# simon-ging/coot-videotext

Measured on AMD Instinct MI355X. Metric: clip-pairs/sec (COOT retrieval train step, whole job), higher is better.
Workload: dtype bf16; 1 GPU; ActivityNet-shaped paper config (anet_coot): 64 videos x 4 clips per GPU, Lc=Lv=80, Ls=16, Lp=64, Dv=2048, Dt=1536, d_model=384; global_batch_videos=64, parallelism=dp1, mode=train, launch=native, deterministic=True, batches=two different synthetic batches in turn

## Files before the change

coot-videotext_amd/csrc/api.hip:

```cpp
#include <stdarg.h>
#include <stdio.h>
#include <string.h>

#include <algorithm>
#include <mutex>
#include <string>
#include <unordered_map>
#include <vector>

#include "../../include/coot_hip.h"
#include "attention.h"
#include "common.h"
#include "fused.h"
#include "gemm.h"
#include "loss.h"
#include "pool.h"
#include "ref_f32.h"
#include "rowops.h"

namespace coot {

static thread_local char g_err[512] = "";
static thread_local hipStream_t g_glob_flush_stream = nullptr;
static thread_local hipEvent_t g_glob_flush_ev = nullptr;
// ... 555 lines not shown
static LayerBufs self_bufs(const LayerS& s, int D) {
  LayerBufs b; b.q = s.qkv; b.ldq = 3 * D; b.k = s.qkv + D; b.ldk = 3 * D; b.v = s.qkv + 2 * D; b.ldv = 3 * D;
  b.ctx = s.ctx; b.r1 = s.r1; b.z1 = s.z1; b.h1 = s.h1; b.a1 = s.a1; b.r2 = s.r2; b.z2 = s.z2; b.lse = s.lse;
  return b;
}
static LayerBufs ctx_bufs(const CtxS& s, int D) {
  LayerBufs b; b.q = s.q; b.ldq = D; b.k = s.kv; b.ldk = 2 * D; b.v = s.kv + D; b.ldv = 2 * D;
  b.ctx = s.cctx; b.r1 = s.r1; b.z1 = s.z1; b.h1 = s.h1; b.a1 = s.a1; b.r2 = s.r2; b.z2 = s.z2; b.lse = s.lse;
  return b;
}

}

using namespace coot;

extern "C" {

const char* coot_last_error(void) { return coot::g_err; }
int coot_version(void) { return COOT_ABI_VERSION; }
int coot_debug_dropout_scales(uint64_t seed, unsigned site, uint64_t idx0, int64_t n, float p, float* out_host) {
  COOT_REQUIRE(out_host && n >= 0 && p > 0.f, "debug_dropout_scales: bad arguments");
  const DropCfg d = mkdrop(1, p, seed, site);
  const unsigned key = drop_key(seed, site);
  for (int64_t i = 0; i < n; ++i) out_host[i] = drop_scale_key(key, idx0 + (uint64_t)i, d.thr, d.inv_keep);
  return 0;
}
int coot_debug_attn_dropout_scales(uint64_t seed, unsigned site, unsigned row32, int Lk, float p, float* out_host) {
  COOT_REQUIRE(out_host && Lk >= 0 && p > 0.f, "debug_attn_dropout_scales: bad arguments");
  const DropCfg d = mkdrop(1, p, seed, site);
  const unsigned key = drop_key(seed, site);
  for (int k = 0; k < Lk; ++k) out_host[k] = attn_drop_scale(key, row32, k, (unsigned)(Lk + 1) >> 1, d.thr, d.inv_keep);
  return 0;
}
int coot_debug_timestamps(void* dev_u64) { g_fz_tstamps = (unsigned long long*)dev_u64; return 0; }
extern "C" void coot_step_stamps_enable(int on);
extern "C" void coot_step_grad_write(int on);
extern "C" void coot_step_det_seg_flush(int on);
extern "C" int coot_step_det_seg_flush_get(void);
extern "C" int coot_internal_stage_hits(void);
extern "C" void coot_step_text_ahead(int on);
extern "C" int coot_step_text_ahead_get(void);
extern "C" int coot_internal_text_ahead_steps(void);
extern "C" int coot_internal_stream_counter(int which);
extern "C++" { namespace coot { int det_bypass_count(); int det_overflow_count(); int det_set_overflow_guard(int on); int det_overflow_guard(); } }
extern "C++" { namespace coot { void set_rt_topk_splits(int n); int get_rt_topk_splits(); void set_rt_few_splits(int n); int get_rt_few_splits(); void set_rt_grouped_splits(int n); int get_rt_grouped_splits(); void set_rt_knn_splits(int n); int get_rt_knn_splits(); void set_rt_comp_blocks_per_wg(int n); int get_rt_comp_blocks_per_wg(); } }
int coot_get_option(const char* name, int* value) {
  if (!value) { set_error("get_option: null result"); return -1; }
  if (!strcmp(name, "tn_dma")) { *value = get_tn_dma(); return 0; }
  if (!strcmp(name, "xcd_order")) { *value = get_xcd_order(); return 0; }
  if (!strcmp(name, "tn_mode")) { *value = get_tn_mode(); return 0; }
  if (!strcmp(name, "stage_hits")) { *value = coot_internal_stage_hits(); return 0; }
  if (!strcmp(name, "text_ahead")) { *value = coot_step_text_ahead_get(); return 0; }
  if (!strcmp(name, "text_ahead_steps")) { *value = coot_internal_text_ahead_steps(); return 0; }
  if (!strcmp(name, "fused_attn_launches")) { *value = fused_attn_launches(); return 0; }
  if (!strcmp(name, "stream_overlap_tests")) { *value = coot_internal_stream_counter(0); return 0; }
  if (!strcmp(name, "stream_candidates_rejected")) { *value = coot_internal_stream_counter(1); return 0; }
  if (!strcmp(name, "stream_unresolved")) { *value = coot_internal_stream_counter(2); return 0; }
  if (!strcmp(name, "operand_f16")) { *value = COOT_OPERAND_IS_F16; return 0; }
  if (!strcmp(name, "det_seg_flush")) { *value = coot_step_det_seg_flush_get(); return 0; }
  if (!strcmp(name, "det_bypasses")) { *value = det_bypass_count(); return 0; }
  if (!strcmp(name, "det_overflows")) { *value = det_overflow_count(); return 0; }
  if (!strcmp(name, "det_overflow_check")) { *value = det_overflow_guard(); return 0; }
  if (!strcmp(name, "rt_topk_splits")) { *value = get_rt_topk_splits(); return 0; }
  if (!strcmp(name, "rt_few_splits")) { *value = get_rt_few_splits(); return 0; }
  if (!strcmp(name, "rt_grouped_splits")) { *value = get_rt_grouped_splits(); return 0; }
  if (!strcmp(name, "rt_knn_splits")) { *value = get_rt_knn_splits(); return 0; }
  if (!strcmp(name, "rt_comp_blocks_per_wg")) { *value = get_rt_comp_blocks_per_wg(); return 0; }
  set_error("get_option: unknown or write-only option %s", name);
  return -2;
}
int coot_set_option(const char* name, int value) {
  if (!strcmp(name, "tn_mode")) { set_tn_mode(value); return 0; }
  if (!strcmp(name, "step_stamps")) { coot_step_stamps_enable(value); return 0; }
  if (!strcmp(name, "fused")) { g_use_fused = value; return 0; }
  if (!strcmp(name, "glob_fused")) { g_use_glob_fused = value; return 0; }
  if (!strcmp(name, "glob_fused_bwd")) { g_use_glob_fused_bwd = value; return 0; }
  if (!strcmp(name, "packed")) { g_use_packed = value; return 0; }
  if (!strcmp(name, "fused_infc")) { g_use_fused_infc = value; return 0; }
  if (!strcmp(name, "fused_attn")) { set_fused_attn(value); return 0; }
  if (!strcmp(name, "tn_dma")) { set_tn_dma(value); return 0; }
  if (!strcmp(name, "pack_lazy")) { g_pack_lazy = value; return 0; }
  if (!strcmp(name, "pack_poison")) { g_pack_poison = value; return 0; }
  if (!strcmp(name, "grad_poison")) { g_grad_poison = value; return 0; }
  if (!strcmp(name, "tn_target_wgs")) { set_tn_target_wgs(value); return 0; }
  if (!strcmp(name, "xcd_order")) { set_xcd_order(value); return 0; }
  if (!strcmp(name, "grad_write")) { coot_step_grad_write(value); return 0; }
  if (!strcmp(name, "det_seg_flush")) { coot_step_det_seg_flush(value); return 0; }
  if (!strcmp(name, "text_ahead")) { coot_step_text_ahead(value); return 0; }
  if (!strcmp(name, "det_overflow_check")) return det_set_overflow_guard(value);
  if (!strcmp(name, "glob_flush_aux")) { g_glob_flush_aux = value; return 0; }
  if (!strcmp(name, "pool_handover")) { g_pool_handover_on = value; return 0; }
  if (!strcmp(name, "cl_col_split")) { set_cl_col_split(value); return 0; }
  if (!strcmp(name, "cl_small")) { set_cl_small(value); return 0; }
  if (!strcmp(name, "fz_debug")) { g_fz_debug = value; return 0; }
  if (!strcmp(name, "fused_min_rows")) { g_fused_min_rows = value; return 0; }
  if (!strcmp(name, "rt_topk_splits")) { set_rt_topk_splits(value); return 0; }
  if (!strcmp(name, "rt_few_splits")) { set_rt_few_splits(value); return 0; }
  if (!strcmp(name, "rt_grouped_splits")) { set_rt_grouped_splits(value); return 0; }
  if (!strcmp(name, "rt_knn_splits")) { set_rt_knn_splits(value); return 0; }
  if (!strcmp(name, "rt_comp_blocks_per_wg")) { set_rt_comp_blocks_per_wg(value); return 0; }
  set_error("unknown option %s", name);
  return -2;
}

int64_t coot_net_param_numel(const coot_net_config* cfg) {
  coot_net_config c; if (norm_cfg(cfg, &c)) return -1;
  NetLayout L; build_layout(c, L); return L.total;
}
int coot_net_param_count(const coot_net_config* cfg) {
  coot_net_config c; if (norm_cfg(cfg, &c)) return -1;
  NetLayout L; build_layout(c, L); return (int)L.entries.size();
}
int coot_net_param_info(const coot_net_config* cfg, int index, char* name, int name_len, int64_t* offset, int64_t shape[4], int* ndim) {
  coot_net_config c; RUN(norm_cfg(cfg, &c));
  NetLayout L; build_layout(c, L);
  COOT_REQUIRE(index >= 0 && index < (int)L.entries.size(), "param index %d out of range", index);
  const PEntry& e = L.entries[index];
  snprintf(name, name_len, "%s", e.name.c_str());
// ... 620 lines not shown
```

coot-videotext_amd/csrc/attention.h:

```cpp
#pragma once
#include "common.h"
#include "rowops.h"

namespace coot {

struct AttnArgs {
  const bf16_t* q = nullptr; long ldq = 0;
  const bf16_t* k = nullptr; long ldk = 0;
  const bf16_t* v = nullptr; long ldv = 0;
  bf16_t* o = nullptr; long ldo = 0;
  float* lse = nullptr;
  const long long* lens = nullptr;
  int Nseq = 0, Lq = 0, Lk = 0, H = 0, dh = 0;
  float scale = 1.0f;
  int xcd_order = 1;
  int Nseq2 = 0, L2 = 0; const long long* lens2 = nullptr; unsigned long long seed2_delta = 0;
  const int* cu = nullptr;
  DropCfg drop;
  const bf16_t* dout = nullptr; long lddo = 0;
  float* delta = nullptr;
  bf16_t* dq = nullptr; long lddq = 0;
  bf16_t* dk = nullptr; long lddk = 0;
  bf16_t* dv = nullptr; long lddv = 0;
};

int launch_attn_fwd(const AttnArgs& a, hipStream_t stream);
int launch_attn_bwd(const AttnArgs& a, hipStream_t stream);
bool attn_short_path(int L);

}
```

coot-videotext_amd/csrc/attention.hip:

```cpp
#include "attention.h"
#include "gemm.h"

namespace coot {

__device__ __forceinline__ float attn_drop(unsigned key, unsigned row, int k, unsigned lk_half, unsigned thr, float inv_keep) {
  return attn_drop_scale(key, row, k, lk_half, thr, inv_keep);
}

constexpr int KC = 64;

template <int DH>
struct AttnSmem {
  static constexpr int RP = DH + 8;
  static constexpr int TP = KC + 8;
};

__device__ __forceinline__ f32x4_t mfma16(s16x4_t a, s16x4_t b, f32x4_t c) {
  return COOT_MFMA_16x16x16(a, b, c);
}
__device__ __forceinline__ s16x4_t pack4(float a, float b, float c, float d) {
  unsigned lo = pack2bf(a, b), hi = pack2bf(c, d);
  s16x4_t r;
  r[0] = (short)(lo & 0xFFFF); r[1] = (short)(lo >> 16); r[2] = (short)(hi & 0xFFFF); r[3] = (short)(hi >> 16);
  return r;
// ... 293 lines not shown
        p[i] = pv * dsc;
        ds[i] = pv * (dp[i] * dsc - delta_s[ql]) * a.scale;
      }
      pf[qt] = pack4(p[0], p[1], p[2], p[3]);
      dsf[qt] = pack4(ds[0], ds[1], ds[2], ds[3]);
    }
#pragma unroll
    for (int dt = 0; dt < NK; ++dt)
#pragma unroll
      for (int qt = 0; qt < 4; ++qt) {
        s16x4_t dotf = *reinterpret_cast<const s16x4_t*>(&dOt[(dt * 16 + lk) * TP + qt * 16 + lg * 4]);
        s16x4_t qtf = *reinterpret_cast<const s16x4_t*>(&Qt[(dt * 16 + lk) * TP + qt * 16 + lg * 4]);
        dvacc[dt] = mfma16(pf[qt], dotf, dvacc[dt]);
        dkacc[dt] = mfma16(dsf[qt], qtf, dkacc[dt]);
      }
  }
#pragma unroll
  for (int dt = 0; dt < NK; ++dt)
#pragma unroll
    for (int i = 0; i < 4; ++i) {
      const int kr = k0 + lg * 4 + i;
      if (kr < Lk) {
        a.dk[(kbase + kr) * a.lddk + h * DH + dt * 16 + lk] = f2bf(dkacc[dt][i]);
        a.dv[(kbase + kr) * a.lddv + h * DH + dt * 16 + lk] = f2bf(dvacc[dt][i]);
      }
    }
}

constexpr int SH_MAXW = 8;

__device__ __forceinline__ s16x4_t tr16(const bf16_t* tile, int pitch, int lane) {
  const int g = lane >> 4, p = lane & 15;
  const bf16_t* addr = tile + (4 * g + (p >> 2)) * pitch + (p & 3) * 4;
  return __builtin_amdgcn_ds_read_tr16_b64_v4i16((s16x4_t __attribute__((address_space(3)))*)(addr));
}

__device__ __forceinline__ bool short_wg(const AttnArgs& a, int& n, int& h) {
  const int id = blockIdx.x, g = id / (8 * a.H), r = id - g * (8 * a.H);
  if (a.xcd_order) { h = r >> 3; n = g * 8 + (r & 7); }
  else { h = id % a.H; n = id / a.H; }
  return n < a.Nseq + a.Nseq2;
}
static inline int short_grid(const AttnArgs& a) { return ((a.Nseq + a.Nseq2 + 7) / 8) * 8 * a.H; }
struct ShortSeq { int n, L, nvalid; long base; unsigned dkey; };
__device__ __forceinline__ ShortSeq short_seq(const AttnArgs& a, int n) {
  ShortSeq s;
  if (a.cu) {
    const bool second = n >= a.Nseq;
    s.n = second ? n - a.Nseq : n;
    s.L = s.nvalid = (int)(second ? a.lens2[s.n] : a.lens[s.n]);
    s.base = a.cu[n];
    s.dkey = a.drop.thr ? drop_site_key(a.drop.seed + (second ? a.seed2_delta : 0ull), a.drop.seed_ptr, a.drop.site) : 0u;
    return s;
  }
  if (n >= a.Nseq) {
    s.n = n - a.Nseq; s.L = a.L2; s.nvalid = (int)a.lens2[s.n]; s.base = (long)a.Nseq * a.Lk + (long)s.n * a.L2;
    s.dkey = a.drop.thr ? drop_site_key(a.drop.seed + a.seed2_delta, a.drop.seed_ptr, a.drop.site) : 0u;
  } else {
    s.n = n; s.L = a.Lk; s.nvalid = (int)a.lens[n]; s.base = (long)n * a.Lk;
    s.dkey = a.drop.thr ? drop_site_key(a.drop.seed, a.drop.seed_ptr, a.drop.site) : 0u;
  }
  return s;
}

template <int DH>
__device__ __forceinline__ void stage_rows(const bf16_t* src, long ld, long rowbase, int L, int L16, int c0, bf16_t* R) {
// ... 90 lines not shown
#pragma unroll
      for (int i = 0; i < 4; ++i) {
        p[i] = __expf(s[kt][i] - mx);
        sum += p[i];
        if (a.drop.thr) {
          const int kidx = kt * 16 + lg * 4 + i;
          p[i] *= attn_drop(dkey, (unsigned)((n * a.H + h) * L + qrow), kidx, (unsigned)(L + 1) >> 1, a.drop.thr, a.drop.inv_keep);
        }
      }
      pf[kt] = pack4(p[0], p[1], p[2], p[3]);
    }
  }
  sum += __shfl_xor(sum, 16, 64);
  sum += __shfl_xor(sum, 32, 64);
  f32x4_t oacc[NK];
#pragma unroll
  for (int dt = 0; dt < NK; ++dt) {
    oacc[dt] = f32x4_t{0, 0, 0, 0};
#pragma unroll
    for (int kt = 0; kt < SH_MAXW; ++kt)
      if (kt < nw) oacc[dt] = mfma16(tr16(&Vs[kt * 16 * RP + dt * 16], RP, lane), pf[kt], oacc[dt]);
  }
  if (qok) {
    const float inv = 1.0f / sum;
#pragma unroll
    for (int dt = 0; dt < NK; ++dt) {
      const u32x2_t pk = {pack2bf(oacc[dt][0] * inv, oacc[dt][1] * inv), pack2bf(oacc[dt][2] * inv, oacc[dt][3] * inv)};
      *reinterpret_cast<u32x2_t*>(a.o + (base + qrow) * a.ldo + h * DH + dt * 16 + lg * 4) = pk;
    }
    if (lg == 0 && a.lse) a.lse[(base + qrow) * a.H + h] = mx + __logf(sum);
  }
}

template <int DH>
__global__ __launch_bounds__(512) void attn_short_bwd_kernel(AttnArgs a) {
  constexpr int RP = AttnSmem<DH>::RP, NK = DH / 16;
  extern __shared__ __attribute__((aligned(16))) bf16_t sh_lds[];
  const int lane = threadIdx.x & 63, wave = threadIdx.x >> 6, nw = blockDim.x >> 6;
  int n, h;
  if (!short_wg(a, n, h)) return;
  const ShortSeq sq = short_seq(a, n);
  n = sq.n;
  const unsigned dkey = sq.dkey;
  const int L = sq.L, L16 = nw * 16;
  bf16_t* Ks = sh_lds;
  bf16_t* Vs = Ks + L16 * RP;
  bf16_t* Qs = Vs + L16 * RP;
  bf16_t* dOs = Qs + L16 * RP;
  float* lse_s = reinterpret_cast<float*>(dOs + L16 * RP);
  float* delta_s = lse_s + L16;
  const int nvalid = sq.nvalid;
  const long base = sq.base;
  const int l15 = lane & 15, lg = lane >> 4;
  const int qrow = wave * 16 + l15;
  const bool qok = qrow < L;
  u32x4_t kst[2], vst[2], qst[2], dst[2];
  stage_load<DH>(a.k, a.ldk, base, L, L16, h * DH, kst);
  stage_load<DH>(a.v, a.ldv, base, L, L16, h * DH, vst);
  stage_load<DH>(a.q, a.ldq, base, L, L16, h * DH, qst);
  stage_load<DH>(a.dout, a.lddo, base, L, L16, h * DH, dst);
  s16x4_t qf[NK], dof[NK], of[NK];
#pragma unroll
  for (int ks = 0; ks < NK; ++ks) {
    qf[ks] = s16x4_t{0, 0, 0, 0}; dof[ks] = qf[ks]; of[ks] = qf[ks];
    if (qok) {
      const long off = h * DH + ks * 16 + lg * 4;
      qf[ks] = *reinterpret_cast<const s16x4_t*>(a.q + (base + qrow) * a.ldq + off);
      dof[ks] = *reinterpret_cast<const s16x4_t*>(a.dout + (base + qrow) * a.lddo + off);
      of[ks] = *reinterpret_cast<const s16x4_t*>(a.o + (base + qrow) * a.ldo + off);
    }
  }
  float lse = 0.f;
  if (qok) lse = a.lse[(base + qrow) * a.H + h];
  stage_store<DH>(Ks, L16, kst);
  stage_store<DH>(Vs, L16, vst);
  stage_store<DH>(Qs, L16, qst);
  stage_store<DH>(dOs, L16, dst);
  float dl = 0.f;
#pragma unroll
  for (int ks = 0; ks < NK; ++ks)
#pragma unroll
    for (int j = 0; j < 4; ++j) dl += bf2f((bf16_t)dof[ks][j]) * bf2f((bf16_t)of[ks][j]);
  dl += __shfl_xor(dl, 16, 64);
  dl += __shfl_xor(dl, 32, 64);
  if (lg == 0) { lse_s[wave * 16 + l15] = lse; delta_s[wave * 16 + l15] = dl; }
  __syncthreads();
  {
    s16x4_t dsf[SH_MAXW];
#pragma unroll
    for (int kt = 0; kt < SH_MAXW; ++kt) {
      if (kt < nw) {
        f32x4_t sv4 = {0, 0, 0, 0}, dp = {0, 0, 0, 0};
#pragma unroll
        for (int ks = 0; ks < NK; ++ks) {
          const s16x4_t kf = *reinterpret_cast<const s16x4_t*>(&Ks[(kt * 16 + l15) * RP + ks * 16 + lg * 4]);
          const s16x4_t vf = *reinterpret_cast<const s16x4_t*>(&Vs[(kt * 16 + l15) * RP + ks * 16 + lg * 4]);
          sv4 = mfma16(kf, qf[ks], sv4);
          dp = mfma16(vf, dof[ks], dp);
        }
        float ds[4];
#pragma unroll
        for (int i = 0; i < 4; ++i) {
          const int kidx = kt * 16 + lg * 4 + i;
          float sv = sv4[i] * a.scale;
          if (kidx >= nvalid) sv = kMaskFill;
          const float p = (kidx < L && qok) ? __expf(sv - lse) : 0.f;
          float dpe = dp[i];
          if (a.drop.thr) {
            dpe *= attn_drop(dkey, (unsigned)((n * a.H + h) * L + qrow), kidx, (unsigned)(L + 1) >> 1, a.drop.thr, a.drop.inv_keep);
          }
          ds[i] = (kidx < nvalid) ? p * (dpe - dl) * a.scale : 0.f;
        }
        dsf[kt] = pack4(ds[0], ds[1], ds[2], ds[3]);
      }
    }
#pragma unroll
    for (int dt = 0; dt < NK; ++dt) {
      f32x4_t dq = {0, 0, 0, 0};
#pragma unroll
      for (int kt = 0; kt < SH_MAXW; ++kt)
        if (kt < nw) dq = mfma16(tr16(&Ks[kt * 16 * RP + dt * 16], RP, lane), dsf[kt], dq);
      if (qok) {
        const u32x2_t pk = {pack2bf(dq[0], dq[1]), pack2bf(dq[2], dq[3])};
        *reinterpret_cast<u32x2_t*>(a.dq + (base + qrow) * a.lddq + h * DH + dt * 16 + lg * 4) = pk;
      }
    }
  }
  const int krow = wave * 16 + l15;
  const bool kin = krow < L, kvalid = krow < nvalid;
  s16x4_t kf[NK], vf[NK];
#pragma unroll
  for (int ks = 0; ks < NK; ++ks) {
    kf[ks] = *reinterpret_cast<const s16x4_t*>(&Ks[krow * RP + ks * 16 + lg * 4]);
    vf[ks] = *reinterpret_cast<const s16x4_t*>(&Vs[krow * RP + ks * 16 + lg * 4]);
  }
  f32x4_t dkacc[NK], dvacc[NK];
#pragma unroll
  for (int dt = 0; dt < NK; ++dt) { dkacc[dt] = f32x4_t{0, 0, 0, 0}; dvacc[dt] = dkacc[dt]; }
#pragma unroll
  for (int qt = 0; qt < SH_MAXW; ++qt) {
    if (qt < nw) {
      f32x4_t sv4 = {0, 0, 0, 0}, dp = {0, 0, 0, 0};
#pragma unroll
      for (int ks = 0; ks < NK; ++ks) {
        const s16x4_t qfr = *reinterpret_cast<const s16x4_t*>(&Qs[(qt * 16 + l15) * RP + ks * 16 + lg * 4]);
        const s16x4_t dofr = *reinterpret_cast<const s16x4_t*>(&dOs[(qt * 16 + l15) * RP + ks * 16 + lg * 4]);
        sv4 = mfma16(qfr, kf[ks], sv4);
        dp = mfma16(dofr, vf[ks], dp);
      }
      float p[4], ds[4];
#pragma unroll
      for (int i = 0; i < 4; ++i) {
        const int qr = qt * 16 + lg * 4 + i;
        const float pv = (kvalid && qr < L) ? __expf(sv4[i] * a.scale - lse_s[qr]) : 0.f;
        float dsc = 1.f;
        if (a.drop.thr) {
          dsc = attn_drop(dkey, (unsigned)((n * a.H + h) * L + qr), krow, (unsigned)(L + 1) >> 1, a.drop.thr, a.drop.inv_keep);
        }
        p[i] = pv * dsc;
        ds[i] = pv * (dp[i] * dsc - delta_s[qr]) * a.scale;
      }
      const s16x4_t pf = pack4(p[0], p[1], p[2], p[3]), dsf = pack4(ds[0], ds[1], ds[2], ds[3]);
#pragma unroll
      for (int dt = 0; dt < NK; ++dt) {
        dvacc[dt] = mfma16(tr16(&dOs[qt * 16 * RP + dt * 16], RP, lane), pf, dvacc[dt]);
        dkacc[dt] = mfma16(tr16(&Qs[qt * 16 * RP + dt * 16], RP, lane), dsf, dkacc[dt]);
      }
    }
  }
  if (kin) {
#pragma unroll
    for (int dt = 0; dt < NK; ++dt) {
      const u32x2_t pk = {pack2bf(dkacc[dt][0], dkacc[dt][1]), pack2bf(dkacc[dt][2], dkacc[dt][3])};
      const u32x2_t pv = {pack2bf(dvacc[dt][0], dvacc[dt][1]), pack2bf(dvacc[dt][2], dvacc[dt][3])};
      *reinterpret_cast<u32x2_t*>(a.dk + (base + krow) * a.lddk + h * DH + dt * 16 + lg * 4) = pk;
      *reinterpret_cast<u32x2_t*>(a.dv + (base + krow) * a.lddv + h * DH + dt * 16 + lg * 4) = pv;
    }
  }
}

template <int DH>
__device__ __forceinline__ void load_row(const bf16_t* p, float (&r)[DH]) {
#pragma unroll
  for (int c = 0; c < DH; c += 4) {
    const s16x4_t v = *reinterpret_cast<const s16x4_t*>(p + c);
#pragma unroll
    for (int j = 0; j < 4; ++j) r[c + j] = bf2f((bf16_t)v[j]);
  }
}
template <int DH>
__device__ __forceinline__ void store_row(bf16_t* p, const float (&r)[DH]) {
#pragma unroll
  for (int c = 0; c < DH; c += 4) {
    const u32x2_t pk = {pack2bf(r[c], r[c + 1]), pack2bf(r[c + 2], r[c + 3])};
    *reinterpret_cast<u32x2_t*>(p + c) = pk;
  }
}
template <int DH>
__global__ __launch_bounds__(256) void attn_q1_fwd_kernel(AttnArgs a) {
// ... 39 lines not shown
    float sv = 0.f;
#pragma unroll
    for (int c = 0; c < DH; ++c) sv += qv[c] * row[c];
    sv *= a.scale;
    if (lane >= nvalid) sv = kMaskFill;
    p = __expf(sv - lse);
    load_row<DH>(a.v + ((long)n * Lk + lane) * a.ldv + h * DH, row);
#pragma unroll
    for (int c = 0; c < DH; ++c) dp += dov[c] * row[c];
    if (a.drop.thr) dr = attn_drop(dkey, (unsigned)(n * a.H + h), lane, (unsigned)(Lk + 1) >> 1, a.drop.thr, a.drop.inv_keep);
  }
  const float pd = p * dr;
  const float delta = wave_sum(pd * dp);
  const float ds = (lane < nvalid) ? p * (dr * dp - delta) * a.scale : 0.f;
  if (lane < Lk) {
#pragma unroll
    for (int c = 0; c < DH; ++c) row[c] = ds * qv[c];
    store_row<DH>(a.dk + ((long)n * Lk + lane) * a.lddk + h * DH, row);
#pragma unroll
    for (int c = 0; c < DH; ++c) row[c] = pd * dov[c];
    store_row<DH>(a.dv + ((long)n * Lk + lane) * a.lddv + h * DH, row);
  }
  float dq = 0.f;
  const bf16_t* kcol = a.k + (long)n * Lk * a.ldk + h * DH + (lane < DH ? lane : 0);
  for (int l = 0; l < Lk; ++l) dq += __shfl(ds, l, 64) * bf2f(kcol[(long)l * a.ldk]);
  if (lane < DH) a.dq[(long)n * a.lddq + h * DH + lane] = f2bf(dq);
}
static bool attn_q1_ok(const AttnArgs& a) { return a.Lq == 1 && a.Lk >= 1 && a.Lk <= 64 && a.Nseq2 == 0; }

static bool attn_short_ok(const AttnArgs& a) {
  return a.Lq == a.Lk && a.Lk <= 16 * SH_MAXW && a.Lk >= 1 && (a.Nseq2 == 0 || (a.L2 >= 1 && a.L2 <= 16 * SH_MAXW));
}
bool attn_short_path(int L) { return L >= 1 && L <= 16 * SH_MAXW; }

template <int DH>
static int attn_fwd_t(const AttnArgs& a_in, hipStream_t st) {
  AttnArgs a = a_in;
  a.xcd_order = get_xcd_order() & 4;
  if (attn_q1_ok(a)) {
    hipLaunchKernelGGL(attn_q1_fwd_kernel<DH>, dim3((a.Nseq * a.H + 3) / 4), dim3(256), 0, st, a);
    COOT_CHECK_LAUNCH("attn_q1_fwd");
    return 0;
  }
  if (attn_short_ok(a)) {
    const int nw = ((a.Nseq2 > 0 && a.L2 > a.Lk ? a.L2 : a.Lk) + 15) / 16;
    hipLaunchKernelGGL(attn_short_fwd_kernel<DH>, dim3(short_grid(a)), dim3(64 * nw), (size_t)2 * nw * 16 * AttnSmem<DH>::RP * sizeof(bf16_t), st, a);
    COOT_CHECK_LAUNCH("attn_short_fwd");
    return 0;
  }
  dim3 grid((a.Lq + 63) / 64, a.H, a.Nseq);
  hipLaunchKernelGGL(attn_fwd_kernel<DH>, grid, dim3(256), 0, st, a);
  COOT_CHECK_LAUNCH("attn_fwd");
  return 0;
}
template <int DH>
__global__ __launch_bounds__(256) void attn_bwd_kernel(AttnArgs a, int nq) {
  if ((int)blockIdx.x < nq) attn_bwd_q_body<DH>(a, (int)blockIdx.x);
  else attn_bwd_kv_body<DH>(a, (int)blockIdx.x - nq);
}
template <int DH>
static int attn_bwd_t(const AttnArgs& a_in, hipStream_t st) {
  AttnArgs a = a_in;
  a.xcd_order = get_xcd_order() & 4;
  if (attn_q1_ok(a)) {
    hipLaunchKernelGGL(attn_q1_bwd_kernel<DH>, dim3((a.Nseq * a.H + 3) / 4), dim3(256), 0, st, a);
    COOT_CHECK_LAUNCH("attn_q1_bwd");
    return 0;
  }
  if (attn_short_ok(a)) {
    const int nw = ((a.Nseq2 > 0 && a.L2 > a.Lk ? a.L2 : a.Lk) + 15) / 16;
    hipLaunchKernelGGL(attn_short_bwd_kernel<DH>, dim3(short_grid(a)), dim3(64 * nw),
                       (size_t)4 * nw * 16 * AttnSmem<DH>::RP * sizeof(bf16_t) + (size_t)2 * nw * 16 * sizeof(float), st, a);
    COOT_CHECK_LAUNCH("attn_short_bwd");
    return 0;
  }
  const int nq = (a.Lq + 63) / 64, nk = (a.Lk + 63) / 64;
  hipLaunchKernelGGL(attn_bwd_kernel<DH>, dim3(nq + nk, a.H, a.Nseq), dim3(256), 0, st, a, nq);
  COOT_CHECK_LAUNCH("attn_bwd");
  return 0;
}

static int attn_check(const AttnArgs& a) {
  COOT_REQUIRE(a.q && a.k && a.v && a.o && a.lens, "attention: null pointer");
  COOT_REQUIRE(a.dh % 16 == 0 && a.dh >= 16 && a.dh <= 64, "attention: d_head=%d unsupported (16,32,48,64)", a.dh);
  COOT_REQUIRE(a.ldq % 4 == 0 && a.ldk % 8 == 0 && a.ldv % 8 == 0 && a.ldo % 4 == 0, "attention: strides must be multiples of 8");
  return 0;
}

int launch_attn_fwd(const AttnArgs& a, hipStream_t st) {
  if (int rc = attn_check(a)) return rc;
  if (a.Nseq <= 0 || a.Lq <= 0) return 0;
  switch (a.dh) {
    case 16: return attn_fwd_t<16>(a, st);
    case 32: return attn_fwd_t<32>(a, st);
    case 48: return attn_fwd_t<48>(a, st);
    default: return attn_fwd_t<64>(a, st);
  }
}

int launch_attn_bwd(const AttnArgs& a, hipStream_t st) {
  if (int rc = attn_check(a)) return rc;
  COOT_REQUIRE(a.dout && a.lse && a.delta && a.dq && a.dk && a.dv, "attention bwd: null pointer");
  COOT_REQUIRE(a.ldq % 8 == 0 && a.lddo % 8 == 0, "attention bwd: strides must be multiples of 8");
  if (a.Nseq <= 0 || a.Lq <= 0) return 0;
  switch (a.dh) {
// ... 9 lines not shown
```

coot-videotext_amd/lib.py:

```python
from __future__ import annotations

import ctypes as C
import os
from typing import List, Tuple

_HERE = os.path.dirname(os.path.abspath(__file__))
OPERAND_ENV = os.environ.get("COOT_OPERAND", "bf16")
if OPERAND_ENV not in ("bf16", "f16"):
    raise RuntimeError(f"COOT_OPERAND={OPERAND_ENV}: bf16 or f16")
LIB_PATH = os.environ.get("COOT_HIP_LIB") or os.path.join(_HERE, "lib", "libcoot_hip_f16.so" if OPERAND_ENV == "f16" else "libcoot_hip.so")

EXPORTS = [
    "coot_last_error", "coot_version", "coot_set_option", "coot_get_option", "coot_debug_timestamps", "coot_debug_step_stamps", "coot_debug_dropout_scales", "coot_debug_attn_dropout_scales", "coot_net_param_numel", "coot_net_param_count",
    "coot_net_param_info", "coot_net_out_dim", "coot_net_wpack_bytes", "coot_net_pack_weights", "coot_nets_pack_weights",
    "coot_net_saved_bytes", "coot_net_scratch_bytes", "coot_net_fwd", "coot_net_bwd", "coot_net_grads_overwrite", "coot_nets_zero_grads", "coot_nets_zero_grads_ex", "coot_debug_written_matrices", "coot_pack_fwd",
    "coot_pack_bwd", "coot_contrastive_scratch_bytes", "coot_contrastive_fwd_bwd", "coot_contrastive_fwd_bwd_part", "coot_contrastive_f32_scratch_bytes", "coot_contrastive_fwd_bwd_f32", "coot_cyclecons_fwd_bwd",
    "coot_gemm_nt", "coot_debug_gemm_nt", "coot_gemm_tn", "coot_gemm_tn_batch", "coot_debug_tn_xcd_map", "coot_debug_clock_monitor", "coot_gemm_tn_workspace_bytes", "coot_ln_fwd", "coot_attn_fwd", "coot_probe_tr16", "coot_timing_enable",
    "coot_timing_collect", "coot_step_workspace_bytes", "coot_train_step", "coot_step_forward", "coot_step_backward",
    "coot_adam_step", "coot_radam_step", "coot_step_update", "coot_step_set_global_done_events", "coot_step_device_state_bytes", "coot_step_set_device_state", "coot_step_loss_scaler_bytes", "coot_step_set_loss_scaler", "coot_step_unscale_grads", "coot_step_grad_clip_bytes", "coot_step_set_grad_clip", "coot_step_grad_norm", "coot_collate_level", "coot_collate_packed", "coot_sample_cycle_indices", "coot_step_set_cycle_indices", "coot_step_input_stage_bytes", "coot_step_set_input_stages", "coot_step_set_next_batch", "coot_contrastive_fwd_bwd_dp", "coot_contrastive_fwd_bwd_dp_blocks", "coot_retrieval_workspace_bytes", "coot_retrieval_ranks", "coot_retrieval_topk_workspace_bytes", "coot_retrieval_topk",
    "coot_retrieval_ranks_part_workspace_bytes", "coot_retrieval_ranks_part", "coot_retrieval_metrics",
    "coot_retrieval_ranks_labeled_workspace_bytes", "coot_retrieval_ranks_labeled",
    "coot_retrieval_row_norms", "coot_retrieval_topk_few_workspace_bytes", "coot_retrieval_topk_few",
    "coot_retrieval_row_norms_h", "coot_retrieval_topk_few_h",
    "coot_retrieval_topk_masked", "coot_retrieval_topk_few_masked", "coot_retrieval_rows_put",
    "coot_retrieval_topk_index_workspace_bytes", "coot_retrieval_topk_index",
    "coot_retrieval_topk_grouped_workspace_bytes", "coot_retrieval_topk_grouped",
    "coot_retrieval_topk_multi_workspace_bytes", "coot_retrieval_topk_multi",
    "coot_retrieval_topk_scoped_workspace_bytes", "coot_retrieval_topk_scoped",
    "coot_retrieval_range_workspace_bytes", "coot_retrieval_range_count", "coot_retrieval_range_scan", "coot_retrieval_range_fill",
    "coot_retrieval_range_tile_workspace_bytes", "coot_retrieval_range_tile_count", "coot_retrieval_range_tile_fill",
    "coot_retrieval_join_count", "coot_retrieval_join_fill",
    "coot_retrieval_cross_join_count", "coot_retrieval_cross_join_fill",
    "coot_retrieval_knn_join_workspace_bytes", "coot_retrieval_knn_join",
    "coot_retrieval_components",
    "coot_det_shadow_bytes", "coot_det_configure", "coot_det_flush", "coot_event_record", "coot_event_wait", "coot_event_handle", "coot_stream_hop",
    "coot_stream_create_concurrent", "coot_stream_destroy", "coot_streams_overlap",
]


class NetConfig(C.Structure):
    _fields_ = [("input_dim", C.c_int), ("hidden_dim", C.c_int), ("num_heads", C.c_int), ("ff_dim", C.c_int),
                ("num_layers", C.c_int), ("use_input_fc", C.c_int), ("use_context", C.c_int),
                ("ctx_num_layers", C.c_int), ("pooler", C.c_int), ("pool_hidden", C.c_int), ("pool_heads", C.c_int),
                ("dropout", C.c_float), ("ctx_dropout", C.c_float), ("pool_dropout", C.c_float), ("dtype", C.c_int)]


class ContrastiveConfig(C.Structure):
    _fields_ = [("margin", C.c_float), ("weight_high", C.c_float), ("weight_high_internal", C.c_float),
                ("weight_low", C.c_float), ("weight_low_internal", C.c_float), ("weight_context", C.c_float),
                ("weight_context_internal", C.c_float)]
# ... 171 lines not shown
    lib.coot_retrieval_join_fill.argtypes = [vp, i32, vp, vp, vp, vp, i32, i32, i32, i32, vp, vp, i64, vp, vp, vp]
    lib.coot_retrieval_cross_join_count.argtypes = [vp, i32, vp, vp, i32, vp, vp, vp, vp, vp, vp, i32, i32, i32, i32, i32, vp, vp]
    lib.coot_retrieval_cross_join_fill.argtypes = [vp, i32, vp, vp, i32, vp, vp, vp, vp, vp, vp, i32, i32, i32, i32, i32, vp, vp, i64, vp, vp, vp]
    lib.coot_retrieval_knn_join_workspace_bytes.argtypes = [i32, i32, i32]
    lib.coot_retrieval_knn_join_workspace_bytes.restype = C.c_size_t
    lib.coot_retrieval_knn_join.argtypes = [vp, i32, vp, vp, i32, vp, vp, vp, vp, vp, i32, i32, i32, i32, i32, vp, vp, vp, C.c_size_t, vp]
    lib.coot_retrieval_components.argtypes = [vp, i32, vp, vp, vp, vp, i32, i32, vp, vp, vp]
    lib.coot_retrieval_ranks_labeled_workspace_bytes.argtypes = [i32, i32, i32]
    lib.coot_retrieval_ranks_labeled_workspace_bytes.restype = C.c_size_t
    lib.coot_retrieval_ranks_labeled.argtypes = [vp, vp, vp, i32, i32, i32, i32, vp, vp, vp, vp, vp, vp, C.c_size_t, vp]
    lib.coot_det_shadow_bytes.restype = sz
    lib.coot_det_shadow_bytes.argtypes = [i32, C.POINTER(sz)]
    lib.coot_det_configure.argtypes = [i32, C.POINTER(vp), C.POINTER(sz), vp, sz, vp]
    lib.coot_det_flush.argtypes = [vp, sz, vp]
    lib.coot_event_record.argtypes = [i32, vp]
    lib.coot_event_wait.argtypes = [i32, vp]
    lib.coot_event_handle.restype = vp
    lib.coot_event_handle.argtypes = [i32]
    lib.coot_stream_hop.argtypes = [vp, vp]
    lib.coot_stream_create_concurrent.argtypes = [C.POINTER(vp), i32, i32, C.POINTER(vp), C.POINTER(i32)]
    lib.coot_stream_destroy.argtypes = [vp]
    lib.coot_streams_overlap.argtypes = [vp, vp]
    lib.coot_gemm_nt.argtypes = [vp, i64, vp, i64, i32, i32, i32, vp, i32, vp, i64, vp, i64, i32, vp]
    lib.coot_debug_gemm_nt.argtypes = [C.POINTER(GemmNtArgs), vp]
    lib.coot_gemm_tn.argtypes = [vp, i64, vp, i64, i32, i32, i32, vp, i64, vp, sz, vp]
    lib.coot_gemm_tn_batch.argtypes = [C.POINTER(TnProblem), i32, vp, sz, vp, vp]
    ip = C.POINTER(i32)
    lib.coot_debug_tn_xcd_map.argtypes = [i32, ip, ip, ip, ip, ip, ip, i32]
    lib.coot_debug_clock_monitor.argtypes = [vp, i32, i32, vp]
    lib.coot_gemm_tn_workspace_bytes.restype = sz
    lib.coot_gemm_tn_workspace_bytes.argtypes = [i32, i32, i32]
    lib.coot_ln_fwd.argtypes = [vp, i32, i32, vp, vp, vp, vp, vp]
    lib.coot_attn_fwd.argtypes = [vp, i32, i32, i32, i32, vp, vp, vp, vp]
    lib.coot_probe_tr16.argtypes = [vp, vp]
    lib.coot_timing_enable.argtypes = [i32]
    lib.coot_timing_collect.argtypes = [i32, C.POINTER(C.c_double), C.POINTER(C.c_double), C.POINTER(i32)]
    scp, sdp, sbp, sxp = C.POINTER(StepConfig), C.POINTER(StepDims), C.POINTER(StepBuffers), C.POINTER(StepBatch)
    lib.coot_step_workspace_bytes.restype = sz
    lib.coot_step_workspace_bytes.argtypes = [scp, sdp]
    lib.coot_train_step.argtypes = [scp, sbp, sxp, sdp, vp, vp, sz, i32, u64, i64, i32, vp, vp, vp]
    lib.coot_step_forward.argtypes = [scp, sbp, sxp, sdp] + [vp] * 6 + [vp, sz, i32, u64, i32, vp, vp, vp]
    lib.coot_step_update.argtypes = [scp, sbp, i64, i32, vp, vp, vp, vp]
    lib.coot_step_set_global_done_events.argtypes = [vp, vp]
    lib.coot_step_device_state_bytes.restype = sz
    lib.coot_step_device_state_bytes.argtypes = []
    lib.coot_step_set_device_state.argtypes = [vp]
    lib.coot_step_loss_scaler_bytes.restype = sz
    lib.coot_step_loss_scaler_bytes.argtypes = []
    lib.coot_step_set_loss_scaler.argtypes = [vp]
    lib.coot_step_unscale_grads.argtypes = [scp, sbp, vp]
    lib.coot_step_grad_clip_bytes.restype = sz
    lib.coot_step_grad_clip_bytes.argtypes = [scp]
    lib.coot_step_set_grad_clip.argtypes = [vp, i32]
    lib.coot_step_grad_norm.argtypes = [scp, sbp, vp]
    lib.coot_collate_level.argtypes = [vp, vp, i64, i64, i64, i32, vp, vp, i32]
    lib.coot_collate_packed.argtypes = [vp, vp, i64, i64, i32, vp, vp, i32]
    lib.coot_sample_cycle_indices.argtypes = [vp, vp, i32, u64, vp, vp]
    lib.coot_step_set_cycle_indices.argtypes = [vp]
    lib.coot_step_input_stage_bytes.argtypes = [scp, sdp]
    lib.coot_step_input_stage_bytes.restype = sz
    lib.coot_step_set_input_stages.argtypes = [vp, vp, sz]
    lib.coot_step_set_next_batch.argtypes = [sxp, sdp]
    lib.coot_contrastive_fwd_bwd_dp.argtypes = [C.POINTER(ContrastiveConfig), i32, i32, i32, i32, C.POINTER(vp * 6), C.POINTER(i64 * 6), vp,
                                                C.POINTER(vp * 6), i32, i32, i32, i32, vp, sz, vp]
    lib.coot_contrastive_fwd_bwd_dp_blocks.argtypes = [C.POINTER(ContrastiveConfig), i32, i32, vp, vp, i32, i32, vp, vp, C.POINTER(i64 * 6), vp,
                                                       C.POINTER(vp * 6), vp, sz, vp]
# ... 48 lines not shown
```

include/coot_hip.h:

```cpp
#ifndef COOT_HIP_H
#define COOT_HIP_H

#include <stddef.h>
#include <stdint.h>

#ifdef __cplusplus
extern "C" {
#endif
#if defined(__GNUC__) || defined(__clang__)
#pragma GCC visibility push(default)
#endif

typedef void* coot_stream_t;

typedef struct coot_net_config {
  int input_dim;
  int hidden_dim;
  int num_heads;
  int ff_dim;
  int num_layers;
  int use_input_fc;
  int use_context;
  int ctx_num_layers;
  int pooler;
// ... 321 lines not shown
  int act;
  const void* aux; int64_t ldaux;
  void* save_pre; int64_t ldpre;
  const void* res; int64_t ldres;
  const float* pe; int pe_L, pe_T0, pe_L2;
  float* colsum;
  float p; uint64_t seed; unsigned site; int64_t drop_ld;
  void* out; int64_t ldc; int out_f32;
  float* part_ws; size_t part_ws_floats;
} coot_gemm_nt_args;
int coot_debug_gemm_nt(const coot_gemm_nt_args* a, coot_stream_t stream);
size_t coot_gemm_tn_workspace_bytes(int T, int Mo, int No);
int coot_gemm_tn(const void* A, int64_t lda, const void* B, int64_t ldb, int T, int Mo, int No, float* C,
                 int64_t ldc, void* workspace, size_t workspace_bytes, coot_stream_t stream);
typedef struct coot_tn_problem {
  const void* A; int64_t lda;
  const void* B; int64_t ldb;
  int T, Mo, No;
  float* C; int64_t ldc;
  float* a_colsum;
  int overwrite;
  int groups;
  int64_t zA, zB, zC;
} coot_tn_problem;
int coot_gemm_tn_batch(const coot_tn_problem* problems, int n, void* workspace, size_t workspace_bytes,
                       uint64_t* stamps, coot_stream_t stream);
int coot_debug_tn_xcd_map(int n, const int* gx, const int* gy, const int* groups, const int* splits, int* out_item,
                          int* out_local, int max_blocks);
int coot_debug_clock_monitor(uint64_t* out, int n, int interval_ticks, coot_stream_t stream);
int coot_ln_fwd(const float* x, int R, int D, const float* gain, const float* bias, void* y_bf16, float* y_f32,
                coot_stream_t stream);
int coot_attn_fwd(const void* qkv, int Nseq, int L, int H, int dh, const int64_t* lens, void* out, float* lse,
                  coot_stream_t stream);
int coot_timing_enable(int on);
int coot_timing_collect(int only_big_k, double* ms, double* flops, int* launches);
int coot_probe_tr16(uint16_t* out, coot_stream_t stream);

#if defined(__GNUC__) || defined(__clang__)
#pragma GCC visibility pop
#endif
#ifdef __cplusplus
}
#endif
#endif
```

Baseline: 223,200 clip-pairs/s.

## Compute attention backward probabilities once and reuse them through shared memory

The short-sequence attention backward kernel gains a variant that computes P and dS once in the query-row pass, stores them into swizzled LDS strips reusing the K/V region, and reads them back with transposed LDS loads for the dK/dV accumulation. This removes the second QK^T/dO·V^T recomputation, the repeated exp and the repeated dropout hashing in the key-row pass. In exchange it adds two block barriers and extra LDS traffic, and it falls back to the old kernel if LDS would exceed 64 KiB. A debug entry point for attention backward and an option toggle are also added.

```diff
diff --git a/coot-videotext_amd/csrc/api.hip b/coot-videotext_amd/csrc/api.hip
--- a/coot-videotext_amd/csrc/api.hip
+++ b/coot-videotext_amd/csrc/api.hip
@@ -611,6 +611,22 @@
   for (int k = 0; k < Lk; ++k) out_host[k] = attn_drop_scale(key, row32, k, (unsigned)(Lk + 1) >> 1, d.thr, d.inv_keep);
   return 0;
 }
+int coot_debug_attn_bwd(const void* qkv, const void* dout, const void* out, const float* lse, int Nseq, int L, const int64_t* lens,
+                        int Nseq2, int L2, const int64_t* lens2, const int* cu_seqlens, int H, int dh, float drop_p, uint64_t seed,
+                        unsigned site, void* dqkv, float* delta_ws, coot_stream_t stream) {
+  COOT_REQUIRE(qkv && dout && out && lse && lens && dqkv && delta_ws, "debug_attn_bwd: null pointer");
+  COOT_REQUIRE(Nseq2 == 0 || lens2, "debug_attn_bwd: a second segment needs its lengths");
+  COOT_REQUIRE(!cu_seqlens || (attn_short_path(L) && (Nseq2 == 0 || attn_short_path(L2))), "debug_attn_bwd: packed rows need the short attention kernels (L <= 128)");
+  const long D = (long)H * dh;
+  AttnArgs a; a.q = (const bf16_t*)qkv; a.k = a.q + D; a.v = a.q + 2 * D; a.ldq = a.ldk = a.ldv = 3 * D;
+  a.o = (bf16_t*)out; a.ldo = D; a.lse = (float*)lse; a.dout = (const bf16_t*)dout; a.lddo = D; a.delta = delta_ws;
+  a.dq = (bf16_t*)dqkv; a.dk = a.dq + D; a.dv = a.dq + 2 * D; a.lddq = a.lddk = a.lddv = 3 * D;
+  a.H = H; a.dh = dh; a.scale = 1.0f / sqrtf((float)dh);
+  a.drop = mkdrop(1, drop_p, seed, site);
+  Segs sg; sg.n = Nseq2 > 0 ? 2 : 1; sg.N[0] = Nseq; sg.L[0] = L; sg.lens[0] = (const long long*)lens;
+  sg.N[1] = Nseq2; sg.L[1] = L2; sg.lens[1] = (const long long*)lens2; sg.cu = cu_seqlens;
+  return attention_all(a, sg, false, true, (hipStream_t)stream);
+}
 int coot_debug_timestamps(void* dev_u64) { g_fz_tstamps = (unsigned long long*)dev_u64; return 0; }
 extern "C" void coot_step_stamps_enable(int on);
 extern "C" void coot_step_grad_write(int on);
@@ -632,6 +648,7 @@
   if (!strcmp(name, "text_ahead")) { *value = coot_step_text_ahead_get(); return 0; }
   if (!strcmp(name, "text_ahead_steps")) { *value = coot_internal_text_ahead_steps(); return 0; }
   if (!strcmp(name, "fused_attn_launches")) { *value = fused_attn_launches(); return 0; }
+  if (!strcmp(name, "attn_bwd_once")) { *value = get_attn_bwd_once(); return 0; }
   if (!strcmp(name, "stream_overlap_tests")) { *value = coot_internal_stream_counter(0); return 0; }
   if (!strcmp(name, "stream_candidates_rejected")) { *value = coot_internal_stream_counter(1); return 0; }
   if (!strcmp(name, "stream_unresolved")) { *value = coot_internal_stream_counter(2); return 0; }
@@ -663,6 +680,7 @@
   if (!strcmp(name, "grad_poison")) { g_grad_poison = value; return 0; }
   if (!strcmp(name, "tn_target_wgs")) { set_tn_target_wgs(value); return 0; }
   if (!strcmp(name, "xcd_order")) { set_xcd_order(value); return 0; }
+  if (!strcmp(name, "attn_bwd_once")) { set_attn_bwd_once(value); return 0; }
   if (!strcmp(name, "grad_write")) { coot_step_grad_write(value); return 0; }
   if (!strcmp(name, "det_seg_flush")) { coot_step_det_seg_flush(value); return 0; }
   if (!strcmp(name, "text_ahead")) { coot_step_text_ahead(value); return 0; }
diff --git a/coot-videotext_amd/csrc/attention.h b/coot-videotext_amd/csrc/attention.h
--- a/coot-videotext_amd/csrc/attention.h
+++ b/coot-videotext_amd/csrc/attention.h
@@ -27,5 +27,7 @@
 int launch_attn_fwd(const AttnArgs& a, hipStream_t stream);
 int launch_attn_bwd(const AttnArgs& a, hipStream_t stream);
 bool attn_short_path(int L);
+void set_attn_bwd_once(int on);
+int get_attn_bwd_once();
 
 }
diff --git a/coot-videotext_amd/csrc/attention.hip b/coot-videotext_amd/csrc/attention.hip
--- a/coot-videotext_amd/csrc/attention.hip
+++ b/coot-videotext_amd/csrc/attention.hip
@@ -349,6 +349,12 @@
 __device__ __forceinline__ s16x4_t tr16(const bf16_t* tile, int pitch, int lane) {
   const int g = lane >> 4, p = lane & 15;
   const bf16_t* addr = tile + (4 * g + (p >> 2)) * pitch + (p & 3) * 4;
+  return __builtin_amdgcn_ds_read_tr16_b64_v4i16((s16x4_t __attribute__((address_space(3)))*)(addr));
+}
+
+__device__ __forceinline__ s16x4_t tr16_swz(const bf16_t* tile, int pitch, int lane) {
+  const int g = lane >> 4, p = lane & 15;
+  const bf16_t* addr = tile + (4 * g + (p >> 2)) * pitch + ((p & 3) ^ g) * 4;
   return __builtin_amdgcn_ds_read_tr16_b64_v4i16((s16x4_t __attribute__((address_space(3)))*)(addr));
 }
 
@@ -505,7 +511,15 @@
   }
 }
 
-template <int DH>
+__host__ __device__ constexpr int attn_bwd_once_pitch(int nw) { return 16 * (nw | 1); }
+template <int DH>
+static size_t attn_short_bwd_lds(int nw, bool once) {
+  const size_t tile = (size_t)nw * 16 * AttnSmem<DH>::RP * sizeof(bf16_t), strip = (size_t)nw * 16 * attn_bwd_once_pitch(nw) * sizeof(bf16_t);
+  if (!once) return 4 * tile + (size_t)2 * nw * 16 * sizeof(float);
+  return 2 * tile + (strip > tile ? 2 * strip : 2 * tile);
+}
+
+template <int DH, bool ONCE>
 __global__ __launch_bounds__(512) void attn_short_bwd_kernel(AttnArgs a) {
   constexpr int RP = AttnSmem<DH>::RP, NK = DH / 16;
   extern __shared__ __attribute__((aligned(16))) bf16_t sh_lds[];
@@ -516,12 +530,15 @@
   n = sq.n;
   const unsigned dkey = sq.dkey;
   const int L = sq.L, L16 = nw * 16;
-  bf16_t* Ks = sh_lds;
+  bf16_t* Ks = ONCE ? sh_lds + 2 * L16 * RP : sh_lds;
   bf16_t* Vs = Ks + L16 * RP;
-  bf16_t* Qs = Vs + L16 * RP;
+  bf16_t* Qs = ONCE ? sh_lds : Vs + L16 * RP;
   bf16_t* dOs = Qs + L16 * RP;
   float* lse_s = reinterpret_cast<float*>(dOs + L16 * RP);
   float* delta_s = lse_s + L16;
+  const int PP = attn_bwd_once_pitch(nw);
+  bf16_t* Ps = Ks;
+  bf16_t* dSs = Ps + L16 * PP;
   const int nvalid = sq.nvalid;
   const long base = sq.base;
   const int l15 = lane & 15, lg = lane >> 4;
@@ -556,10 +573,11 @@
     for (int j = 0; j < 4; ++j) dl += bf2f((bf16_t)dof[ks][j]) * bf2f((bf16_t)of[ks][j]);
   dl += __shfl_xor(dl, 16, 64);
   dl += __shfl_xor(dl, 32, 64);
-  if (lg == 0) { lse_s[wave * 16 + l15] = lse; delta_s[wave * 16 + l15] = dl; }
+  if (!ONCE && lg == 0) { lse_s[wave * 16 + l15] = lse; delta_s[wave * 16 + l15] = dl; }
   __syncthreads();
   {
     s16x4_t dsf[SH_MAXW];
+    s16x4_t pst[ONCE ? SH_MAXW : 1], dsst[ONCE ? SH_MAXW : 1];
 #pragma unroll
     for (int kt = 0; kt < SH_MAXW; ++kt) {
       if (kt < nw) {
@@ -571,20 +589,27 @@
           sv4 = mfma16(kf, qf[ks], sv4);
           dp = mfma16(vf, dof[ks], dp);
         }
-        float ds[4];
+        float ds[4], pb[4], dsb[4];
 #pragma unroll
         for (int i = 0; i < 4; ++i) {
           const int kidx = kt * 16 + lg * 4 + i;
           float sv = sv4[i] * a.scale;
           if (kidx >= nvalid) sv = kMaskFill;
           const float p = (kidx < L && qok) ? __expf(sv - lse) : 0.f;
-          float dpe = dp[i];
+          float dpe = dp[i], dsc = 1.f;
           if (a.drop.thr) {
-            dpe *= attn_drop(dkey, (unsigned)((n * a.H + h) * L + qrow), kidx, (unsigned)(L + 1) >> 1, a.drop.thr, a.drop.inv_keep);
+            dsc = attn_drop(dkey, (unsigned)((n * a.H + h) * L + qrow), kidx, (unsigned)(L + 1) >> 1, a.drop.thr, a.drop.inv_keep);
+            dpe *= dsc;
           }
           ds[i] = (kidx < nvalid) ? p * (dpe - dl) * a.scale : 0.f;
+          if constexpr (ONCE) {
+            const float pv = (kidx < nvalid && qok) ? __expf(__fmaf_rn(sv4[i], a.scale, -lse)) : 0.f;
+            pb[i] = pv * dsc;
+            dsb[i] = pv * __fmaf_rn(dp[i], dsc, -dl) * a.scale;
+          }
         }
         dsf[kt] = pack4(ds[0], ds[1], ds[2], ds[3]);
+        if constexpr (ONCE) { pst[kt] = pack4(pb[0], pb[1], pb[2], pb[3]); dsst[kt] = pack4(dsb[0], dsb[1], dsb[2], dsb[3]); }
       }
     }
 #pragma unroll
@@ -598,46 +623,73 @@
         *reinterpret_cast<u32x2_t*>(a.dq + (base + qrow) * a.lddq + h * DH + dt * 16 + lg * 4) = pk;
       }
     }
+    if constexpr (ONCE) {
+      __syncthreads();
+#pragma unroll
+      for (int kt = 0; kt < SH_MAXW; ++kt) {
+        if (kt < nw) {
+          const int off = qrow * PP + kt * 16 + ((lg ^ (l15 >> 2)) << 2);
+          *reinterpret_cast<s16x4_t*>(&Ps[off]) = pst[kt];
+          *reinterpret_cast<s16x4_t*>(&dSs[off]) = dsst[kt];
+        }
+      }
+      __syncthreads();
+    }
   }
   const int krow = wave * 16 + l15;
   const bool kin = krow < L, kvalid = krow < nvalid;
-  s16x4_t kf[NK], vf[NK];
-#pragma unroll
-  for (int ks = 0; ks < NK; ++ks) {
-    kf[ks] = *reinterpret_cast<const s16x4_t*>(&Ks[krow * RP + ks * 16 + lg * 4]);
-    vf[ks] = *reinterpret_cast<const s16x4_t*>(&Vs[krow * RP + ks * 16 + lg * 4]);
-  }
   f32x4_t dkacc[NK], dvacc[NK];
 #pragma unroll
   for (int dt = 0; dt < NK; ++dt) { dkacc[dt] = f32x4_t{0, 0, 0, 0}; dvacc[dt] = dkacc[dt]; }
-#pragma unroll
-  for (int qt = 0; qt < SH_MAXW; ++qt) {
-    if (qt < nw) {
-      f32x4_t sv4 = {0, 0, 0, 0}, dp = {0, 0, 0, 0};
-#pragma unroll
-      for (int ks = 0; ks < NK; ++ks) {
-        const s16x4_t qfr = *reinterpret_cast<const s16x4_t*>(&Qs[(qt * 16 + l15) * RP + ks * 16 + lg * 4]);
-        const s16x4_t dofr = *reinterpret_cast<const s16x4_t*>(&dOs[(qt * 16 + l15) * RP + ks * 16 + lg * 4]);
-        sv4 = mfma16(qfr, kf[ks], sv4);
-        dp = mfma16(dofr, vf[ks], dp);
-      }
-      float p[4], ds[4];
-#pragma unroll
-      for (int i = 0; i < 4; ++i) {
-        const int qr = qt * 16 + lg * 4 + i;
-        const float pv = (kvalid && qr < L) ? __expf(sv4[i] * a.scale - lse_s[qr]) : 0.f;
-        float dsc = 1.f;
-        if (a.drop.thr) {
-          dsc = attn_drop(dkey, (unsigned)((n * a.H + h) * L + qr), krow, (unsigned)(L + 1) >> 1, a.drop.thr, a.drop.inv_keep);
-        }
-        p[i] = pv * dsc;
-        ds[i] = pv * (dp[i] * dsc - delta_s[qr]) * a.scale;
-      }
-      const s16x4_t pf = pack4(p[0], p[1], p[2], p[3]), dsf = pack4(ds[0], ds[1], ds[2], ds[3]);
-#pragma unroll
-      for (int dt = 0; dt < NK; ++dt) {
-        dvacc[dt] = mfma16(tr16(&dOs[qt * 16 * RP + dt * 16], RP, lane), pf, dvacc[dt]);
-        dkacc[dt] = mfma16(tr16(&Qs[qt * 16 * RP + dt * 16], RP, lane), dsf, dkacc[dt]);
+  if constexpr (ONCE) {
+#pragma unroll
+    for (int qt = 0; qt < SH_MAXW; ++qt) {
+      if (qt < nw) {
+        const s16x4_t pf = tr16_swz(&Ps[qt * 16 * PP + wave * 16], PP, lane);
+        const s16x4_t dsf = tr16_swz(&dSs[qt * 16 * PP + wave * 16], PP, lane);
+#pragma unroll
+        for (int dt = 0; dt < NK; ++dt) {
+          dvacc[dt] = mfma16(tr16(&dOs[qt * 16 * RP + dt * 16], RP, lane), pf, dvacc[dt]);
+          dkacc[dt] = mfma16(tr16(&Qs[qt * 16 * RP + dt * 16], RP, lane), dsf, dkacc[dt]);
+        }
+      }
+    }
+  } else {
+    s16x4_t kf[NK], vf[NK];
+#pragma unroll
+    for (int ks = 0; ks < NK; ++ks) {
+      kf[ks] = *reinterpret_cast<const s16x4_t*>(&Ks[krow * RP + ks * 16 + lg * 4]);
+      vf[ks] = *reinterpret_cast<const s16x4_t*>(&Vs[krow * RP + ks * 16 + lg * 4]);
+    }
+#pragma unroll
+    for (int qt = 0; qt < SH_MAXW; ++qt) {
+      if (qt < nw) {
+        f32x4_t sv4 = {0, 0, 0, 0}, dp = {0, 0, 0, 0};
+#pragma unroll
+        for (int ks = 0; ks < NK; ++ks) {
+          const s16x4_t qfr = *reinterpret_cast<const s16x4_t*>(&Qs[(qt * 16 + l15) * RP + ks * 16 + lg * 4]);
+          const s16x4_t dofr = *reinterpret_cast<const s16x4_t*>(&dOs[(qt * 16 + l15) * RP + ks * 16 + lg * 4]);
+          sv4 = mfma16(qfr, kf[ks], sv4);
+          dp = mfma16(dofr, vf[ks], dp);
+        }
+        float p[4], ds[4];
+#pragma unroll
+        for (int i = 0; i < 4; ++i) {
+          const int qr = qt * 16 + lg * 4 + i;
+          const float pv = (kvalid && qr < L) ? __expf(sv4[i] * a.scale - lse_s[qr]) : 0.f;
+          float dsc = 1.f;
+          if (a.drop.thr) {
+            dsc = attn_drop(dkey, (unsigned)((n * a.H + h) * L + qr), krow, (unsigned)(L + 1) >> 1, a.drop.thr, a.drop.inv_keep);
+          }
+          p[i] = pv * dsc;
+          ds[i] = pv * (dp[i] * dsc - delta_s[qr]) * a.scale;
+        }
+        const s16x4_t pf = pack4(p[0], p[1], p[2], p[3]), dsf = pack4(ds[0], ds[1], ds[2], ds[3]);
+#pragma unroll
+        for (int dt = 0; dt < NK; ++dt) {
+          dvacc[dt] = mfma16(tr16(&dOs[qt * 16 * RP + dt * 16], RP, lane), pf, dvacc[dt]);
+          dkacc[dt] = mfma16(tr16(&Qs[qt * 16 * RP + dt * 16], RP, lane), dsf, dkacc[dt]);
+        }
       }
     }
   }
@@ -743,6 +795,9 @@
   return a.Lq == a.Lk && a.Lk <= 16 * SH_MAXW && a.Lk >= 1 && (a.Nseq2 == 0 || (a.L2 >= 1 && a.L2 <= 16 * SH_MAXW));
 }
 bool attn_short_path(int L) { return L >= 1 && L <= 16 * SH_MAXW; }
+static int g_attn_bwd_once = 1;
+void set_attn_bwd_once(int on) { g_attn_bwd_once = on != 0; }
+int get_attn_bwd_once() { return g_attn_bwd_once; }
 
 template <int DH>
 static int attn_fwd_t(const AttnArgs& a_in, hipStream_t st) {
@@ -780,8 +835,11 @@
   }
   if (attn_short_ok(a)) {
     const int nw = ((a.Nseq2 > 0 && a.L2 > a.Lk ? a.L2 : a.Lk) + 15) / 16;
-    hipLaunchKernelGGL(attn_short_bwd_kernel<DH>, dim3(short_grid(a)), dim3(64 * nw),
-                       (size_t)4 * nw * 16 * AttnSmem<DH>::RP * sizeof(bf16_t) + (size_t)2 * nw * 16 * sizeof(float), st, a);
+    if (g_attn_bwd_once && attn_short_bwd_lds<DH>(nw, true) <= 65536) {
+      hipLaunchKernelGGL((attn_short_bwd_kernel<DH, true>), dim3(short_grid(a)), dim3(64 * nw), attn_short_bwd_lds<DH>(nw, true), st, a);
+    } else {
+      hipLaunchKernelGGL((attn_short_bwd_kernel<DH, false>), dim3(short_grid(a)), dim3(64 * nw), attn_short_bwd_lds<DH>(nw, false), st, a);
+    }
     COOT_CHECK_LAUNCH("attn_short_bwd");
     return 0;
   }
diff --git a/coot-videotext_amd/lib.py b/coot-videotext_amd/lib.py
--- a/coot-videotext_amd/lib.py
+++ b/coot-videotext_amd/lib.py
@@ -15,7 +15,7 @@
     "coot_net_param_info", "coot_net_out_dim", "coot_net_wpack_bytes", "coot_net_pack_weights", "coot_nets_pack_weights",
     "coot_net_saved_bytes", "coot_net_scratch_bytes", "coot_net_fwd", "coot_net_bwd", "coot_net_grads_overwrite", "coot_nets_zero_grads", "coot_nets_zero_grads_ex", "coot_debug_written_matrices", "coot_pack_fwd",
     "coot_pack_bwd", "coot_contrastive_scratch_bytes", "coot_contrastive_fwd_bwd", "coot_contrastive_fwd_bwd_part", "coot_contrastive_f32_scratch_bytes", "coot_contrastive_fwd_bwd_f32", "coot_cyclecons_fwd_bwd",
-    "coot_gemm_nt", "coot_debug_gemm_nt", "coot_gemm_tn", "coot_gemm_tn_batch", "coot_debug_tn_xcd_map", "coot_debug_clock_monitor", "coot_gemm_tn_workspace_bytes", "coot_ln_fwd", "coot_attn_fwd", "coot_probe_tr16", "coot_timing_enable",
+    "coot_gemm_nt", "coot_debug_gemm_nt", "coot_gemm_tn", "coot_gemm_tn_batch", "coot_debug_tn_xcd_map", "coot_debug_clock_monitor", "coot_gemm_tn_workspace_bytes", "coot_ln_fwd", "coot_attn_fwd", "coot_debug_attn_bwd", "coot_probe_tr16", "coot_timing_enable",
     "coot_timing_collect", "coot_step_workspace_bytes", "coot_train_step", "coot_step_forward", "coot_step_backward",
     "coot_adam_step", "coot_radam_step", "coot_step_update", "coot_step_set_global_done_events", "coot_step_device_state_bytes", "coot_step_set_device_state", "coot_step_loss_scaler_bytes", "coot_step_set_loss_scaler", "coot_step_unscale_grads", "coot_step_grad_clip_bytes", "coot_step_set_grad_clip", "coot_step_grad_norm", "coot_collate_level", "coot_collate_packed", "coot_sample_cycle_indices", "coot_step_set_cycle_indices", "coot_step_input_stage_bytes", "coot_step_set_input_stages", "coot_step_set_next_batch", "coot_contrastive_fwd_bwd_dp", "coot_contrastive_fwd_bwd_dp_blocks", "coot_retrieval_workspace_bytes", "coot_retrieval_ranks", "coot_retrieval_topk_workspace_bytes", "coot_retrieval_topk",
     "coot_retrieval_ranks_part_workspace_bytes", "coot_retrieval_ranks_part", "coot_retrieval_metrics",
@@ -253,6 +253,7 @@
     lib.coot_gemm_tn_workspace_bytes.argtypes = [i32, i32, i32]
     lib.coot_ln_fwd.argtypes = [vp, i32, i32, vp, vp, vp, vp, vp]
     lib.coot_attn_fwd.argtypes = [vp, i32, i32, i32, i32, vp, vp, vp, vp]
+    lib.coot_debug_attn_bwd.argtypes = [vp, vp, vp, vp, i32, i32, vp, i32, i32, vp, vp, i32, i32, f32, u64, C.c_uint, vp, vp, vp]
     lib.coot_probe_tr16.argtypes = [vp, vp]
     lib.coot_timing_enable.argtypes = [i32]
     lib.coot_timing_collect.argtypes = [i32, C.POINTER(C.c_double), C.POINTER(C.c_double), C.POINTER(i32)]
diff --git a/include/coot_hip.h b/include/coot_hip.h
--- a/include/coot_hip.h
+++ b/include/coot_hip.h
@@ -377,6 +377,9 @@
                 coot_stream_t stream);
 int coot_attn_fwd(const void* qkv, int Nseq, int L, int H, int dh, const int64_t* lens, void* out, float* lse,
                   coot_stream_t stream);
+int coot_debug_attn_bwd(const void* qkv, const void* dout, const void* out, const float* lse, int Nseq, int L,
+                        const int64_t* lens, int Nseq2, int L2, const int64_t* lens2, const int* cu_seqlens, int H, int dh,
+                        float drop_p, uint64_t seed, unsigned site, void* dqkv, float* delta_ws, coot_stream_t stream);
 int coot_timing_enable(int on);
 int coot_timing_collect(int only_big_k, double* ms, double* flops, int* launches);
 int coot_probe_tr16(uint16_t* out, coot_stream_t stream);
```

New measurement: 222,700 clip-pairs/s. Within noise of the previous version (-0.2%).
